# CPJKU/beat_this

Measured on AMD Instinct MI355X. Metric: audio-seconds processed/sec, higher is better.
Workload: dtype f32 activations, f16x3 products (3 x f16 MFMA on hi+lo operand halves, f32 accumulate); main-layer attention P.V: 2 x, probabilities as fp16 hi parts

## Files before the change

### beat_this_amd/_lib.py

```python
from __future__ import annotations

import ctypes as C
import os
import subprocess

import torch

PKG_DIR = os.path.dirname(os.path.abspath(__file__))
LIB_PATH = os.path.join(PKG_DIR, "libbeat_this_amd.so")
if os.environ.get("BT_DEV") == "1" and os.environ.get("BT_LIB_PATH"):
    LIB_PATH = os.environ["BT_LIB_PATH"]
SOURCES = ["gemm.hip", "gemm2.hip", "gemm3.hip", "gemm_mx8.hip", "attn.hip", "attn2.hip", "fused.hip", "fused2.hip", "qkv_front.hip", "frontend.hip", "logmel.hip",
           "tail.hip", "dbn.hip", "metrics.hip", "loss.hip", "data.hip", "train.hip", "train_front.hip", "optim.hip", "engine.hip"]
HEADERS = ["common.h", "chain.h", "kernels.h", "dropout.h", "train_common.h", "train_mixed.inc", "train_front_mixed.inc", "attn_x3_loop.inc", "attn_hq2_loop.inc", os.path.join("..", "..", "include", "beat_this_amd.h")]

BT_OK, BT_ERR_ARG, BT_ERR_HIP, BT_ERR_WORKSPACE = 0, -1, -2, -3
ABI_VERSION = 600
PREC_F32, PREC_HALF, PREC_F32X3 = 0, 1, 3
OPT_X3_ATTN_P16, OPT_X3_GEMM_FP8, OPT_WS_GUARD = 1, 2, 3
MAX_LAYERS = 32
PROFILE_CATEGORIES = ["stem", "qkv_gemm", "attn_flash", "out_gemm", "ff1_gemm", "ff2_gemm", "conv_gemm",
                      "linear_gemm", "head", "ff_fused", "attn_freq_fused", "layer_tail"]

GEMM_EPI_STORE, GEMM_EPI_RESID, GEMM_EPI_QKV = 0, 1, 2
# ... 183 lines not shown
    "bt_audio2beats_plan": (C.c_int, [C.c_void_p, C.c_int64, C.c_int, C.c_int, C.c_int, C.POINTER(A2BPlan)]),
    "bt_audio2beats_enqueue": (C.c_int, [C.c_void_p, C.c_void_p, C.c_int, C.POINTER(LogmelTables), C.c_void_p, C.c_int64, C.c_int, C.c_int,
                                         C.c_void_p, C.c_int, C.c_void_p, C.c_size_t, C.c_void_p, C.c_int]),
    "bt_profile_begin": (None, [C.c_void_p]),
    "bt_profile_end": (C.c_int, [C.c_void_p, C.c_void_p, C.c_void_p, C.c_int]),
    "bt_resample_batch": (C.c_int, [C.c_void_p, C.c_void_p, C.c_int, C.c_int64, C.c_int, C.c_int, C.c_void_p, C.c_int,
                                    C.c_void_p]),
    "bt_logmel_batch": (C.c_int, [C.c_void_p, C.POINTER(LogmelTables), C.c_void_p, C.c_int, C.c_int64, C.c_void_p]),
    "bt_split_chunks_batch": (C.c_int, [C.c_void_p, C.c_void_p, C.c_void_p, C.c_int, C.c_int, C.c_void_p]),
    "bt_aggregate_batch": (C.c_int, [C.c_void_p, C.c_void_p, C.c_void_p, C.c_void_p, C.c_void_p, C.c_int, C.c_int64,
                                     C.c_int, C.c_int, C.c_void_p, C.c_void_p]),
    "bt_peaks_batch": (C.c_int, [C.c_void_p, C.c_void_p, C.c_void_p, C.c_int, C.c_void_p, C.c_void_p]),
    "bt_peaks_host": (C.c_int, [C.c_void_p, C.c_int64, C.c_void_p, C.POINTER(C.c_int32)]),
    "bt_gemm": (C.c_int, [C.c_void_p, C.c_int, C.POINTER(GemmArgs)]),
    "bt_attention": (C.c_int, [C.c_void_p, C.c_int, C.POINTER(AttnArgs)]),
    "bt_gemm3": (C.c_int, [C.c_void_p, C.POINTER(Gemm3Args)]),
    "bt_gemm_mx8": (C.c_int, [C.c_void_p, C.c_void_p, C.c_void_p, C.c_void_p, C.c_void_p, C.c_void_p, C.c_int, C.c_int, C.c_int, C.c_int64]),
    "bt_attn_frag_blocks": (C.c_int, [C.c_int]),
    "bt_attention_frag": (C.c_int, [C.c_void_p, C.POINTER(AttnFragArgs)]),
    "bt_qkv_front": (C.c_int, [C.c_void_p, C.c_int, C.POINTER(PairWeights), C.c_void_p, C.c_void_p, C.c_int, C.c_int, C.c_int,
                               C.c_void_p, C.c_void_p, C.c_void_p, C.c_void_p, C.c_int]),
    "bt_outff_fused": (C.c_int, [C.c_void_p, C.c_int, C.POINTER(PairWeights), C.c_void_p, C.c_void_p, C.c_int64, C.c_void_p]),
    "bt_attnff_fused": (C.c_int, [C.c_void_p, C.c_int, C.POINTER(PairWeights), C.c_void_p, C.c_void_p, C.c_int64]),
    "bt_layer_tail": (C.c_int, [C.c_void_p, C.POINTER(PairWeights), C.c_int, C.c_void_p, C.c_void_p, C.c_int64, C.c_void_p,
                                C.c_void_p]),
    "bt_ff_fused": (C.c_int, [C.c_void_p, C.c_int, C.POINTER(PairWeights), C.c_void_p, C.c_int64]),
    "bt_dbn_tables": (C.c_int, [C.c_double, C.c_double, C.c_double, C.c_int, C.c_double, C.c_double, C.c_double, C.c_void_p,
                                C.c_int, C.c_void_p, C.POINTER(C.c_size_t)]),
    "bt_dbn_workspace_bytes": (C.c_size_t, [C.c_void_p, C.c_int, C.c_int64]),
    "bt_dbn_decode": (C.c_int, [C.c_void_p, C.c_void_p, C.c_void_p, C.c_void_p, C.c_int, C.c_void_p, C.c_int, C.c_int64,
                                C.c_void_p, C.c_void_p, C.c_size_t]),
    "bt_dbn_viterbi": (C.c_int, [C.c_void_p, C.c_void_p, C.c_void_p, C.c_int, C.c_void_p, C.c_int64, C.c_void_p, C.c_void_p,
                                 C.c_void_p, C.c_size_t]),
    "bt_dbn_viterbi_host": (C.c_int, [C.c_void_p, C.c_int, C.c_void_p, C.c_int64, C.c_void_p, C.c_void_p]),
    "bt_dbn_host": (C.c_int, [C.c_void_p, C.c_void_p, C.c_void_p, C.c_int64, C.c_void_p, C.POINTER(C.c_int32)]),
    "bt_dbn_host_act": (C.c_int, [C.c_void_p, C.c_void_p, C.c_int64, C.c_void_p, C.POINTER(C.c_int32)]),
    "bt_beat_metrics_workspace_bytes": (C.c_size_t, [C.c_int, C.c_int64, C.c_int64]),
    "bt_beat_metrics": (C.c_int, [C.c_void_p, C.c_void_p, C.c_void_p, C.c_void_p, C.c_void_p, C.c_int, C.c_double, C.c_double,
                                  C.c_double, C.c_double, C.c_double, C.c_void_p, C.c_size_t, C.c_void_p]),
    "bt_beat_metrics_host": (C.c_int, [C.c_void_p, C.c_void_p, C.c_void_p, C.c_void_p, C.c_int, C.c_double, C.c_double,
                                       C.c_double, C.c_double, C.c_double, C.c_void_p]),
    "bt_bce_loss_workspace_bytes": (C.c_size_t, [C.c_int, C.c_int64]),
    "bt_bce_loss": (C.c_int, [C.c_void_p, C.c_int, C.c_int, C.c_float, C.c_void_p, C.c_void_p, C.c_int, C.c_void_p, C.c_int,
                              C.c_void_p, C.c_int, C.c_void_p, C.c_int, C.c_int64, C.c_int64, C.c_void_p, C.c_size_t,
                              C.c_void_p, C.c_void_p, C.c_void_p, C.c_int, C.c_void_p, C.c_void_p]),
    "bt_bce_loss_backward": (C.c_int, [C.c_void_p, C.c_void_p, C.c_int64, C.c_void_p, C.c_int, C.c_int64, C.c_void_p, C.c_int]),
# ... 188 lines not shown
```

### beat_this_amd/csrc/engine.hip

```cpp
#include <algorithm>
#include <cmath>
#include <cstddef>
#include <cstdio>
#include <cstring>
#include <mutex>
#include <string>
#include <vector>

#include "../../include/beat_this_amd.h"
#include "common.h"
#include "kernels.h"


static thread_local std::string g_err;
static int bt_set_error(int code, const std::string& msg) {
  g_err = msg;
  return code;
}
int bt_set_error_external(int code, const char* msg) { return bt_set_error(code, msg); }

namespace prof {
struct Rec { int cat; hipEvent_t a, b; };
struct State { bool on = false; std::vector<Rec> recs; };
struct Scope {
// ... 2 lines not shown
    if (!st) return;
    Rec r; r.cat = cat;
    (void)hipEventCreate(&r.a); (void)hipEventCreate(&r.b);
    (void)hipEventRecord(r.a, s);
    idx = st->recs.size(); st->recs.push_back(r);
  }
  ~Scope() { if (st) (void)hipEventRecord(st->recs[idx].b, s); }
};
}

struct FwdGraph { int B, T, prec; void* ws; hipGraphExec_t exec; unsigned long stamp; };

struct bt_engine {
  bt_model_desc d;
  prof::State prof;
  std::mutex mu;
  std::vector<FwdGraph> graphs;
  unsigned long graph_clock = 0;
  hipStream_t cap_stream = nullptr;
  std::vector<int> warm;
  int x3_attn_p16 = 1;
  int x3_gemm_fp8 = 0;
  int ws_guard = 0;
};
enum { CAT_STEM = 0, CAT_QKV, CAT_ATTN_FLASH, CAT_OUT, CAT_FF1, CAT_FF2, CAT_CONV, CAT_LINEAR,
       CAT_HEAD, CAT_FF_FUSED, CAT_ATTN_FREQ_FUSED, CAT_LAYER_TAIL, CAT_COUNT };

namespace {

inline size_t align_up(size_t v, size_t a) { return (v + a - 1) / a * a; }

struct Workspace {
  float* xa; float* xb; float* xm; float* gates; void* xmb;
  void* qkv; void* ao; void* hid;
  void* qf; void* kf; void* vf; float* gates_h; int nbp;
  float* ssq[2];
  int* status;
  int* fix_mask;
  size_t total;
};

Workspace carve(char* base, int B, int T, int D, int ff_mult, int prec, size_t guard = 0,
                std::vector<int64_t>* regions = nullptr) {
  const bool x3 = prec == BT_PREC_F32X3;
  if (x3) prec = BT_PREC_F32;
  const size_t es = prec == BT_PREC_F32 ? 4 : 2;
  const size_t bt = (size_t)B * T;
// ... 414 lines not shown
  *out = e;
  return BT_OK;
}
static void drop_graphs(bt_engine* e) {
  for (auto& g : e->graphs) (void)hipGraphExecDestroy(g.exec);
  e->graphs.clear();
  e->warm.clear();
}
void bt_engine_destroy(bt_engine* e) {
  if (!e) return;
  for (auto& r : e->prof.recs) { (void)hipEventDestroy(r.a); (void)hipEventDestroy(r.b); }
  drop_graphs(e);
  if (e->cap_stream) (void)hipStreamDestroy(e->cap_stream);
  delete e;
}

int bt_engine_set_option(bt_engine* e, int option, int value) {
  if (!e) return bt_set_error(BT_ERR_ARG, "null argument");
  std::lock_guard<std::mutex> lock(e->mu);
  if (option == BT_OPT_X3_ATTN_P16 && value >= 0 && value <= 3) { if (e->x3_attn_p16 != value) drop_graphs(e); e->x3_attn_p16 = value; return BT_OK; }
  if (option == BT_OPT_X3_GEMM_FP8 && value >= 0 && value <= 2) { if (e->x3_gemm_fp8 != value) drop_graphs(e); e->x3_gemm_fp8 = value; return BT_OK; }
  if (option == BT_OPT_WS_GUARD && value >= 0 && value % 256 == 0) { if (e->ws_guard != value) drop_graphs(e); e->ws_guard = value; return BT_OK; }
  return bt_set_error(BT_ERR_ARG, "unknown engine option / value");
}
int bt_engine_get_option(const bt_engine* e, int option, int* value) {
  if (!e || !value) return bt_set_error(BT_ERR_ARG, "null argument");
  if (option == BT_OPT_X3_ATTN_P16) { *value = e->x3_attn_p16; return BT_OK; }
  if (option == BT_OPT_X3_GEMM_FP8) { *value = e->x3_gemm_fp8; return BT_OK; }
  if (option == BT_OPT_WS_GUARD) { *value = e->ws_guard; return BT_OK; }
  return bt_set_error(BT_ERR_ARG, "unknown engine option");
}

size_t bt_workspace_bytes(const bt_engine* e, int B, int T, int prec) {
  if (!e || B <= 0 || T <= 0) return 0;
  return carve(nullptr, B, T, e->d.transformer_dim, e->d.ff_mult, prec, (size_t)e->ws_guard).total;
}

int bt_workspace_regions(const bt_engine* e, int B, int T, int prec, int64_t* begin_end, int max) {
  if (!e || B <= 0 || T <= 0 || max < 0 || (max > 0 && !begin_end)) return bt_set_error(BT_ERR_ARG, "bad argument to bt_workspace_regions");
  if (prec != BT_PREC_F32 && prec != BT_PREC_HALF && prec != BT_PREC_F32X3) return bt_set_error(BT_ERR_ARG, "unknown precision");
  std::vector<int64_t> r;
  carve(nullptr, B, T, e->d.transformer_dim, e->d.ff_mult, prec, (size_t)e->ws_guard, &r);
  const int n = (int)(r.size() / 2);
  for (int i = 0; i < std::min(n, max); ++i) { begin_end[2 * i] = r[2 * i]; begin_end[2 * i + 1] = r[2 * i + 1]; }
  return n;
}
// ... 314 lines not shown
  size_t off = 0;
  auto take = [&](size_t bytes) { size_t o = off; off += align_up(bytes, 256); return o; };
  plan->forward_bytes = bt_workspace_bytes(e, plan->B, plan->T, prec);
  plan->off_forward = take(plan->forward_bytes);
  plan->off_chunks = take((size_t)plan->B * plan->T * 128 * 4);
  plan->off_chunk_logits = take((size_t)2 * plan->B * plan->T * 4);
  plan->off_wave22 = take(up == down ? 0 : (size_t)n22 * 4);
  plan->off_spect = take((size_t)n * 128 * 4);
  plan->off_logits = take((size_t)2 * n * 4);
  plan->off_result = take((size_t)plan->result_words * 4);
  plan->ws_bytes = off;
  return BT_OK;
}

int bt_audio2beats_enqueue(bt_engine* e, void* stream, int prec, const bt_logmel_tables* t, const float* d_audio, int64_t n_in,
                           int up, int down, const float* d_filter, int half_len, void* d_ws, size_t ws_bytes, int32_t* h_result,
                           int use_graph) {
  if (!e || !t || !d_audio || !d_ws || !h_result) return bt_set_error(BT_ERR_ARG, "null argument");
  if (up != down && (!d_filter || half_len < 0)) return bt_set_error(BT_ERR_ARG, "resampling needs the polyphase filter");
  bt_a2b_plan pl;
  if (int rc = bt_audio2beats_plan(e, n_in, up, down, prec, &pl)) return rc;
  if (pl.ws_bytes > ws_bytes) return bt_set_error(BT_ERR_WORKSPACE, "workspace too small (bt_audio2beats_plan)");
  std::lock_guard<std::mutex> lock(e->mu);
  const int max_T = e->d.rope_len > 0 ? e->d.rope_len : 1536;
  if (pl.T > max_T) return bt_set_error(BT_ERR_ARG, "chunk longer than the rotary table");
  hipStream_t s = (hipStream_t)stream;
  char* ws = (char*)d_ws;
  float* wave22 = (float*)(ws + pl.off_wave22);
  float* spect = (float*)(ws + pl.off_spect);
  float* chunks = (float*)(ws + pl.off_chunks);
  float* cb = (float*)(ws + pl.off_chunk_logits);
  float* cd = cb + (size_t)pl.B * pl.T;
  float* beat = (float*)(ws + pl.off_logits);
  float* downb = beat + pl.n_frames;
  int32_t* res = (int32_t*)(ws + pl.off_result);
  void* fws = ws + pl.off_forward;
  const int border = 6;
  const float* a22 = d_audio;
  if (up != down) {
    const bt_span_t one{d_audio, (long)n_in, 0, (long)pl.n22};
    LAUNCH(launch_resample(one, nullptr, 1, (long)pl.n22, up, down, d_filter, half_len, wave22, s), "resample");
    a22 = wave22;
  }
  LogmelP lp;
  fill_logmel(lp, t, spect);
  lp.one = bt_span_t{a22, (long)pl.n22, 0, (long)pl.n_frames};
// ... 202 lines not shown
```

### beat_this_amd/csrc/fused2.hip

```cpp
#include <type_traits>

#include "chain.h"
#include "kernels.h"

namespace {

typedef __amdgpu_buffer_rsrc_t rsrc_t;
typedef __attribute__((address_space(3))) void* lptr_t;
DEVI unsigned pk2_hf(float a, float b) {
  const hfx2 t = {(hf)a, (hf)b};
  return __builtin_bit_cast(unsigned, t);
}

template <typename T, int C>
struct WRing {
  static constexpr int KT = C / 32;
  static constexpr int TILE_B = 32 * 32 * (int)sizeof(T);
  static constexpr int STEP_B = 2 * KT * TILE_B;
#ifndef BT_F2_NST_HL128
#define BT_F2_NST_HL128 2
#endif
#ifndef BT_F2_NST_HL64
#define BT_F2_NST_HL64 2
#endif
  static constexpr bool HL = sizeof(T) == 4 && !std::is_same<T, float>::value;
  static constexpr int NST = C == 128 ? (HL ? BT_F2_NST_HL128 : 3) : (HL && C == 64 ? BT_F2_NST_HL64 : 4);
  static constexpr int CH = STEP_B / 4096;
  rsrc_t rs;
  char* lds;
  int tid, wave, total;
  DEVI void issue(int s) {
    if (s >= total) return;
    char* dst = lds + (s % NST) * STEP_B + wave * 1024;
#pragma unroll
    for (int i = 0; i < CH; ++i)
      __builtin_amdgcn_raw_ptr_buffer_load_lds(rs, (lptr_t)(dst + i * 4096), 16, tid * 16, s * STEP_B + i * 4096, 0, 0);
  }
  DEVI void prologue() {
#pragma unroll
    for (int s = 0; s < NST - 1; ++s) issue(s);
  }
  DEVI const char* acquire(int s) {
    const int ahead = min(NST - 2, total - 1 - s);
    if (ahead >= 2) asm volatile("s_waitcnt vmcnt(%0) lgkmcnt(0)" ::"n"(2 * CH) : "memory");
    else if (ahead == 1) asm volatile("s_waitcnt vmcnt(%0) lgkmcnt(0)" ::"n"(CH) : "memory");
    else asm volatile("s_waitcnt vmcnt(0) lgkmcnt(0)" ::: "memory");
    __builtin_amdgcn_s_barrier();
    issue(s + NST - 1);
    return lds + (s % NST) * STEP_B;
  }
};

template <typename T, int C, bool STORE_X = true>
DEVI void ff_tail(WRing<T, C>& ws, int step0, float (&xn)[C / 32][16], const float* b1s, const float* b2,
                  float* xrow, hf* xbrow, bool ok, int lane, int g) {
  constexpr int KT = C / 32, HB = 4 * C / 32;
  constexpr int TILE_B = WRing<T, C>::TILE_B;
  float ss = 0.f;
#pragma unroll
  for (int kt = 0; kt < KT; ++kt)
#pragma unroll
    for (int r = 0; r < 16; ++r) ss = fmaf(xn[kt][r], xn[kt][r], ss);
  ss += __shfl_xor(ss, 32);
  constexpr float PW = OpScale<T>::PW;
  const float scale = sqrtf((float)C) / fmaxf(sqrtf(ss), 1e-12f) * PW;
  Frag<T> xf[KT];
#pragma unroll
  for (int kt = 0; kt < KT; ++kt) xf[kt] = pack_frag<T>(xn[kt]);
  f32x16 acc2[KT];
#pragma unroll
  for (int mt = 0; mt < KT; ++mt)
#pragma unroll
    for (int r = 0; r < 16; ++r) acc2[mt][r] = xn[mt][r] * (1.f / PW);
#pragma unroll 1
  for (int hb = 0; hb < HB; ++hb) {
    const char* wb = ws.acquire(step0 + hb);
    f32x16 acc1;
    zero16(acc1);
#pragma unroll
    for (int kt = 0; kt < KT; ++kt) mma32(acc1, lds_frag<T>(wb + kt * TILE_B, lane), xf[kt]);
    float h[16];
#pragma unroll
    for (int a = 0; a < 4; ++a) {
      const f32x4 b = *reinterpret_cast<const f32x4*>(b1s + hb * 32 + 8 * a + 4 * g);
#pragma unroll
      for (int j = 0; j < 4; ++j) h[4 * a + j] = gelu_t<T>(fmaf(acc1[4 * a + j], scale, b[j]));
    }
    const Frag<T> hf = pack_frag<T>(h);
#pragma unroll
    for (int mt = 0; mt < KT; ++mt) mma32(acc2[mt], lds_frag<T>(wb + (KT + mt) * TILE_B, lane), hf);
  }
#pragma unroll
  for (int mt = 0; mt < KT; ++mt) {
    f32x4 v[4];
#pragma unroll
    for (int a = 0; a < 4; ++a) {
      const int f0 = mt * 32 + 8 * a + 4 * g;
      const f32x4 b = *reinterpret_cast<const f32x4*>(b2 + f0);
#pragma unroll
      for (int j = 0; j < 4; ++j) v[a][j] = fmaf(acc2[mt][4 * a + j], PW, b[j]);
      if constexpr (STORE_X) {
        if (ok) *reinterpret_cast<f32x4*>(xrow + f0) = v[a];
      }
    }
    if (xbrow) {
      typedef __attribute__((ext_vector_type(4))) unsigned int u32x4;
      if constexpr (std::is_same<T, hl>::value) {
#pragma unroll
        for (int k = 0; k < 2; ++k) {
          unsigned xh[2], xl[2], yh[2], yl[2];
#pragma unroll
          for (int i = 0; i < 2; ++i) {
            split_hl4(v[2 * k][2 * i], v[2 * k][2 * i + 1], v[2 * k + 1][2 * i], v[2 * k + 1][2 * i + 1], xh[i], xl[i], yh[i], yl[i]);
// ... 1 lines not shown
          auto h0 = __builtin_amdgcn_permlane32_swap(xh[0], yh[0], false, false);
          auto h1 = __builtin_amdgcn_permlane32_swap(xh[1], yh[1], false, false);
          auto l0 = __builtin_amdgcn_permlane32_swap(xl[0], yl[0], false, false);
          auto l1 = __builtin_amdgcn_permlane32_swap(xl[1], yl[1], false, false);
          if (ok) {
            *reinterpret_cast<u32x4*>(xbrow + mt * 64 + 16 * k + 8 * g) = u32x4{h0[0], h1[0], h0[1], h1[1]};
            *reinterpret_cast<u32x4*>(xbrow + mt * 64 + 32 + 16 * k + 8 * g) = u32x4{l0[0], l1[0], l0[1], l1[1]};
          }
        }
      } else {
#pragma unroll
      for (int k = 0; k < 2; ++k) {
        const unsigned x0 = pk2_hf(v[2 * k][0], v[2 * k][1]), x1 = pk2_hf(v[2 * k][2], v[2 * k][3]);
        const unsigned y0 = pk2_hf(v[2 * k + 1][0], v[2 * k + 1][1]), y1 = pk2_hf(v[2 * k + 1][2], v[2 * k + 1][3]);
        auto r0 = __builtin_amdgcn_permlane32_swap(x0, y0, false, false);
        auto r1 = __builtin_amdgcn_permlane32_swap(x1, y1, false, false);
        if (ok) *reinterpret_cast<u32x4*>(xbrow + mt * 32 + 16 * k + 8 * g) = u32x4{r0[0], r1[0], r0[1], r1[1]};
      }
      }
    }
  }
}

template <typename T, int C, bool STORE_X = true>
__global__ __launch_bounds__(256) void outff_fused_kernel(const FusedOutFFP p) {
  constexpr int KT = C / 32, HB = 4 * C / 32;
  constexpr int TILE_B = WRing<T, C>::TILE_B, STEP_B = WRing<T, C>::STEP_B, NST = WRing<T, C>::NST;
  __shared__ __attribute__((aligned(16))) char wl[NST * STEP_B + 4 * C * 4];
  float* b1s = reinterpret_cast<float*>(wl + NST * STEP_B);
  const int tid = threadIdx.x, lane = tid & 63, wave = __builtin_amdgcn_readfirstlane(tid >> 6);
  const int g = lane >> 5, lr = lane & 31;
  const long tok = ((long)blockIdx.x * 4 + wave) * 32 + lr;
  const bool ok = tok < p.M;
  float* xrow = p.x + (ok ? tok : 0) * C;
  for (int i = tid; i < 4 * C; i += 256) b1s[i] = p.b1[i];

  const T* arow = reinterpret_cast<const T*>(p.ao) + (ok ? tok : 0) * C;
  Frag<T> af[KT];
#pragma unroll
  for (int kt = 0; kt < KT; ++kt) af[kt] = ldg_frag<T>(arow + kt * 32 + 16 * g);
  float xn[KT][16];
#pragma unroll
  for (int mt = 0; mt < KT; ++mt)
#pragma unroll
    for (int a = 0; a < 4; ++a) {
      const f32x4 v = ok ? *reinterpret_cast<const f32x4*>(xrow + mt * 32 + 8 * a + 4 * g) : f32x4{0.f, 0.f, 0.f, 0.f};
#pragma unroll
      for (int j = 0; j < 4; ++j) xn[mt][4 * a + j] = v[j];
    }
  WRing<T, C> ws;
  ws.rs = __builtin_amdgcn_make_buffer_rsrc(const_cast<void*>(p.wfrag), 0, (unsigned)((KT + HB) * STEP_B), 0x00020000);
  ws.lds = wl; ws.tid = tid; ws.wave = wave; ws.total = KT + HB;
  __syncthreads();
  asm volatile("s_waitcnt vmcnt(0)" ::: "memory");
  ws.prologue();
#pragma unroll
  for (int mt = 0; mt < KT; ++mt) {
    const char* wb = ws.acquire(mt);
    f32x16 acc;
    zero16(acc);
#pragma unroll
    for (int kt = 0; kt < KT; ++kt) mma32(acc, lds_frag<T>(wb + kt * TILE_B, lane), af[kt]);
#pragma unroll
    for (int r = 0; r < 16; ++r) xn[mt][r] = fmaf(acc[r], OpScale<T>::PW, xn[mt][r]);
  }
  hf* xbrow = p.xb ? reinterpret_cast<hf*>(p.xb) + tok * C * (std::is_same<T, hl>::value ? 2 : 1) : nullptr;
  ff_tail<T, C, STORE_X>(ws, KT, xn, b1s, p.b2, xrow, xbrow, ok, lane, g);
}

template <typename T, int C>
__global__ __launch_bounds__(256) void attnff_fused_kernel(const FusedAttnFFP p) {
  constexpr int KT = C / 32;
  constexpr int H = C / 32;
  constexpr int F = 1024 / C;
  constexpr int HB = 4 * C / 32;
  constexpr int TILE_B = WRing<T, C>::TILE_B, STEP_B = WRing<T, C>::STEP_B, NST = WRing<T, C>::NST;
  __shared__ __attribute__((aligned(16))) char wl[NST * STEP_B + 4 * C * 4];
  float* b1s = reinterpret_cast<float*>(wl + NST * STEP_B);
  const int tid = threadIdx.x, lane = tid & 63, wave = __builtin_amdgcn_readfirstlane(tid >> 6);
  const int g = lane >> 5, lr = lane & 31;
  const long tok = ((long)blockIdx.x * 4 + wave) * 32 + lr;
  const bool ok = tok < p.M;
  float* xrow = p.x + (ok ? tok : 0) * C;
  for (int i = tid; i < 4 * C; i += 256) b1s[i] = p.b1[i];

  float ss = 0.f;
  Frag<T> xf[KT];
#pragma unroll
  for (int kt = 0; kt < KT; ++kt) xf[kt] = ldx_frag<T>(xrow + kt * 32 + 16 * g, ok, ss);
  ss += __shfl_xor(ss, 32);
  constexpr float PW = OpScale<T>::PW, PA = OpScale<T>::PA;
  const float scale = sqrtf((float)C) / fmaxf(sqrtf(ss), 1e-12f) * PW;
  float sk[16];
#pragma unroll
  for (int r = 0; r < 16; ++r) sk[r] = __shfl(scale, crow(r, g));
  const int pos = (int)(tok & (F - 1));
  f32x2 cs[8];
#pragma unroll
  for (int a = 0; a < 4; ++a)
#pragma unroll
    for (int b = 0; b < 2; ++b)
      cs[2 * a + b] = *reinterpret_cast<const f32x2*>(p.rope + ((long)pos * 16 + 4 * a + 2 * g + b) * 2);
  float bg[H];
#pragma unroll
  for (int hd = 0; hd < H; ++hd) bg[hd] = p.b_gates[hd];
  WRing<T, C> ws;
  ws.rs = __builtin_amdgcn_make_buffer_rsrc(const_cast<void*>(p.wfrag), 0, (unsigned)((1 + 2 * H + HB) * STEP_B), 0x00020000);
  ws.lds = wl; ws.tid = tid; ws.wave = wave; ws.total = 1 + 2 * H + HB;
  __syncthreads();
  asm volatile("s_waitcnt vmcnt(0)" ::: "memory");
  ws.prologue();

  float gate[H];
  {
    const char* wb = ws.acquire(0);
    f32x16 ag;
    zero16(ag);
#pragma unroll
    for (int kt = 0; kt < KT; ++kt) mma32(ag, lds_frag<T>(wb + kt * TILE_B, lane), xf[kt]);
#pragma unroll
    for (int hd = 0; hd < H; ++hd) {
      float v = __shfl(ag[hd], lr);
      gate[hd] = sigmoidf(fmaf(v, scale, bg[hd]));
    }
  }

  f32x16 acco[KT];
#pragma unroll
  for (int mt = 0; mt < KT; ++mt) zero16(acco[mt]);
// ... 57 lines not shown
      float o[16];
#pragma unroll
      for (int r = 0; r < 16; ++r) o[r] = ao[r] * fin;
      const Frag<T> of = pack_frag<T>(o);
#pragma unroll
      for (int mt = 0; mt < KT; ++mt) mma32(acco[mt], lds_frag<T>(wb + (KT + mt) * TILE_B, lane), of);
    }
  }
  f32x4 xv[KT][4];
#pragma unroll
  for (int mt = 0; mt < KT; ++mt)
#pragma unroll
    for (int a = 0; a < 4; ++a)
      xv[mt][a] = ok ? *reinterpret_cast<const f32x4*>(xrow + mt * 32 + 8 * a + 4 * g) : f32x4{0.f, 0.f, 0.f, 0.f};
  asm volatile("s_waitcnt vmcnt(0)" ::: "memory");
  __builtin_amdgcn_sched_barrier(0);
  float xn[KT][16];
#pragma unroll
  for (int mt = 0; mt < KT; ++mt)
#pragma unroll
    for (int a = 0; a < 4; ++a)
#pragma unroll
      for (int j = 0; j < 4; ++j) xn[mt][4 * a + j] = fmaf(acco[mt][4 * a + j], PW, xv[mt][a][j]);
  ff_tail<T, C>(ws, 1 + 2 * H, xn, b1s, p.b2, xrow, nullptr, ok, lane, g);
}

template <typename T>
int launch_outff_t(const FusedOutFFP& p, hipStream_t s) {
  dim3 grid((unsigned)((p.M + 127) / 128)), block(256);
  if constexpr (std::is_same<T, hl>::value) {
    if (p.shadow_only) {
      if (!p.xb) return -2;
      switch (p.C) {
        case 64: hipLaunchKernelGGL((outff_fused_kernel<T, 64, false>), grid, block, 0, s, p); break;
        case 128: hipLaunchKernelGGL((outff_fused_kernel<T, 128, false>), grid, block, 0, s, p); break;
        default: return -2;
      }
      return (int)hipGetLastError();
    }
  } else if (p.shadow_only) {
    return -2;
  }
  switch (p.C) {
    case 32: hipLaunchKernelGGL((outff_fused_kernel<T, 32>), grid, block, 0, s, p); break;
    case 64: hipLaunchKernelGGL((outff_fused_kernel<T, 64>), grid, block, 0, s, p); break;
    case 128: hipLaunchKernelGGL((outff_fused_kernel<T, 128>), grid, block, 0, s, p); break;
    default: return -2;
  }
  return (int)hipGetLastError();
}
template <typename T>
int launch_attnff_t(const FusedAttnFFP& p, hipStream_t s) {
  dim3 grid((unsigned)((p.M + 127) / 128)), block(256);
  switch (p.C) {
    case 32: hipLaunchKernelGGL((attnff_fused_kernel<T, 32>), grid, block, 0, s, p); break;
    case 64: hipLaunchKernelGGL((attnff_fused_kernel<T, 64>), grid, block, 0, s, p); break;
    case 128: hipLaunchKernelGGL((attnff_fused_kernel<T, 128>), grid, block, 0, s, p); break;
    default: return -2;
  }
  return (int)hipGetLastError();
}

}

int launch_outff_fused(const FusedOutFFP& p, int prec, hipStream_t s) {
  if (p.M <= 0) return -2;
  if (prec == BT_PREC_F32X3) return BT_HALF_IS_BF16 ? -2 : launch_outff_t<hl>(p, s);
  return prec == BT_PREC_F32 ? launch_outff_t<float>(p, s) : launch_outff_t<hf>(p, s);
}
int launch_attnff_fused(const FusedAttnFFP& p, int prec, hipStream_t s) {
  if (p.M <= 0) return -2;
  if (prec == BT_PREC_F32X3) return BT_HALF_IS_BF16 ? -2 : launch_attnff_t<hl>(p, s);
  return prec == BT_PREC_F32 ? launch_attnff_t<float>(p, s) : launch_attnff_t<hf>(p, s);
}
```

### beat_this_amd/csrc/kernels.h

```cpp
#pragma once
#include <hip/hip_runtime.h>
#include <stdint.h>

#ifndef BT_PREC_F32
#define BT_PREC_F32 0
#define BT_PREC_HALF 1
#endif
#ifndef BT_PREC_F32X3
#define BT_PREC_F32X3 3
#endif

enum {
  GEMM_EPI_STORE = 0,
  GEMM_EPI_RESID = 1,
  GEMM_EPI_QKV = 2
};
enum {
  GEMM_F_RMS = 1,
  GEMM_F_BIAS = 2,
  GEMM_F_GELU = 4,
  GEMM_F_OUT_F32 = 8,
  GEMM_F_A_F32 = 16,
  GEMM_F_CONV = 32,
  GEMM_F_ROWMAP = 64
// ... 96 lines not shown
  float* x; long M; int C;
  const void* wfrag;
  const float* b1; const float* b2;
  void* xb;
};
int launch_ff_fused(const FusedFFP& p, int prec, hipStream_t s);

struct FusedOutFFP {
  float* x; long M; int C;
  const void* ao;
  const void* wfrag;
  const float* b1; const float* b2;
  void* xb;
  int shadow_only;
};
int launch_outff_fused(const FusedOutFFP& p, int prec, hipStream_t s);
struct FusedAttnFFP {
  float* x; long M; int C;
  const float* b_gates; const float* rope;
  const void* wfrag;
  const float* b1; const float* b2;
};
int launch_attnff_fused(const FusedAttnFFP& p, int prec, hipStream_t s);

struct LayerTailP {
  float* x; long M; int C; int hidden;
  const void* ao;
  const void* wfrag;
  const float* b1; const float* b2;
  void* xb;
  float* ssq_out;
};
bool layer_tail_supported(int C, int hidden);
int launch_layer_tail(const LayerTailP& p, hipStream_t s);

struct StemP {
  const float* spect;
  float* x;
  const float* bn1_scale; const float* bn1_shift;
  const float* w;
  const float* bias;
  int B, T;
};
int launch_stem(const StemP& p, hipStream_t s);

struct HeadP {
// ... 37 lines not shown
```

### beat_this_amd/pack.py

```python
from __future__ import annotations

import collections
import ctypes as C
import math
import threading

import torch

from . import _lib, tables

LOG2E = 1.4426950408889634
BN_EPS = 1e-5


def perm32(w: torch.Tensor) -> torch.Tensor:
    idx = torch.tensor([(r & 3) + 8 * (r >> 2) + 4 * g for g in range(2) for r in range(16)])
    n, k = w.shape
    return w.reshape(n, k // 32, 32)[:, :, idx].reshape(n, k).contiguous()


def fragment_tiles(w: torch.Tensor) -> torch.Tensor:
    r, k = w.shape
    t = w.reshape(r // 32, 32, k // 32, 2, 16)
    return t.permute(0, 2, 3, 1, 4).reshape(r // 32, k // 32, 64, 16)
# ... 256 lines not shown
            t = tail_fragment_major(sd[pa + "to_out.0.weight"].to(torch.float32), perm32(w1),
                                    perm32(sd[pf + "net.4.weight"].to(torch.float32)))
            t = t.to(_lib.half_torch_dtype()).to(self.device)
            self._keep.append(t)
            pw.w_tail_frag = t.data_ptr()


class PackedPair:

    def __init__(self, sd: dict, attn_prefix: str, ff_prefix: str, dim: int, device):
        self.device = torch.device(device)
        self._keep: list[torch.Tensor] = []
        self.weights = _lib.PairWeights()
        sd = {k: v.detach().to("cpu", torch.float32) for k, v in sd.items()}
        PackedModel._pair(self, self.weights, sd, attn_prefix, ff_prefix, dim, x3=True)

    _f32 = PackedModel._f32
    _mat = PackedModel._mat
    _hl32 = PackedModel._hl32
    _hl8 = PackedModel._hl8
    _x3_stream = PackedModel._x3_stream


class Engine:

    def __init__(self, packed: PackedModel):
        self.packed = packed
        self.device = packed.device
        h = C.c_void_p()
        _lib.check(_lib.lib().bt_engine_create(C.byref(packed.desc), C.byref(h)))
        self._h = h
        self._ws = collections.OrderedDict()
        self._graphs = collections.OrderedDict()
        self._graph_ws = {}
        self._a2b_ws = {}
        self._graphs_ok = True
        self.profiling = False
        self._lock = threading.Lock()
        self.last_fallbacks = 0

    def __del__(self):
        try:
            if getattr(self, "_h", None):
                _lib.lib().bt_engine_destroy(self._h)
                self._h = None
        except Exception:
            pass

    MAX_WORKSPACES = 4
    SHRINK_AFTER = 8
    OPTIONS = {"x3_attn_p16": 1, "x3_gemm_fp8": 2, "ws_guard": 3}

    def set_options(self, opts: dict) -> None:
        for name in opts:
            if name not in self.OPTIONS:
                raise ValueError(f"unknown engine option {name!r} (known: {sorted(self.OPTIONS)})")
        if int(opts.get("x3_gemm_fp8", 0)) > 0:
# ... 103 lines not shown
    def forward_unit(self, x: torch.Tensor, prec: int, unit: int, index: int, out_shape) -> torch.Tensor:
        _lib.require_gpu(x, "sub-module input")
        B, T = int(x.shape[0]), int(x.shape[1])
        if B == 0 or T == 0:
            raise ValueError("empty batch")
        if prec == _lib.PREC_F32X3:
            prec = _lib.PREC_F32
        x = x.to(torch.float32).contiguous()
        self.ensure_positions(T)
        ws = self._workspace(_lib.lib().bt_workspace_bytes(self._h, B, T, prec))
        out = torch.empty(tuple(out_shape), dtype=torch.float32, device=self.device)
        with torch.cuda.device(self.device):
            _lib.check(_lib.lib().bt_forward_unit(self._h, _lib.stream_ptr(self.device), prec, unit, index, x.data_ptr(),
                                                  out.data_ptr(), B, T, ws.data_ptr(), ws.numel()))
        return out

    GRAPH_MAX_CHUNKS = 11
    GRAPH_T = 1500
    GRAPH_MAX_ENTRIES = 12

    def graph_forward(self, B: int, T: int, prec: int):
        if not self._graphs_ok or T != self.GRAPH_T or B > self.GRAPH_MAX_CHUNKS or self.profiling:
            return None
        stream = torch.cuda.current_stream(self.device)
        key = (stream, B, T, prec)
        e = self._graphs.pop(key, None)
        if e is None:
            try:
                e = _GraphEntry(self, B, T, prec, stream)
            except Exception as err:
                self._graphs_ok = False
                self._graph_error = repr(err)
                return None
        cache = self._graphs
        cache[key] = e
        while len(cache) > self.GRAPH_MAX_ENTRIES:
            cache.popitem(last=False)
        return e

    def _graph_workspace(self, stream, need: int) -> torch.Tensor:
        pool = self._graph_ws
        ws = pool.get(stream)
        if ws is None or ws.numel() < need:
            ws = pool[stream] = torch.empty(need, dtype=torch.uint8, device=self.device)
        return ws

# ... 67 lines not shown
```

### include/beat_this_amd.h

```cpp
#ifndef BEAT_THIS_AMD_H
#define BEAT_THIS_AMD_H
#include <stddef.h>
#include <stdint.h>

#ifdef __cplusplus
extern "C" {
#endif

#define BT_OK 0
#define BT_ERR_ARG (-1)
#define BT_ERR_HIP (-2)
#define BT_ERR_WORKSPACE (-3)

#define BT_PREC_F32 0
#define BT_PREC_HALF 1

#define BT_PREC_F32X3 3

#define BT_MAX_LAYERS 32

typedef struct bt_engine bt_engine;

typedef struct {
  int32_t dim, heads;
// ... 232 lines not shown
  int32_t n_seq, L, heads, inner, nbp, o_div; int64_t o_outer, o_inner, o_tok;
  int32_t x3, out_f32; int32_t* status;
  int32_t* scratch;
} bt_attn_frag_args;
int bt_gemm_mx8(void* stream, const void* d_A, const void* d_SA, const void* d_W, const void* d_SW, float* d_out, int M, int N,
                int K, int64_t ldo);

typedef struct {
  const void* A; int64_t lda; int32_t M, K; const void* W; int32_t N, epi; const float* bias;
  const float* ssq_in; int32_t ssq_parts; void* out; int64_t ldo; float* x; int64_t ldx; void* xb; float* ssq_out;
  int32_t n_seq, L, nbp, heads; const float* rope; void* qf; void* kf; void* vf; float* gates; const float* b_gates;
  int32_t no_resid;
  int32_t gelu, conv_C2, conv_T, conv_F;
  int32_t x3; int32_t* status;
} bt_gemm3_args;
int bt_gemm3(void* stream, const bt_gemm3_args* a);
int bt_attn_frag_blocks(int L);
int bt_attention_frag(void* stream, const bt_attn_frag_args* a);
int bt_qkv_front(void* stream, int prec, const bt_pair_weights* w, const float* d_rope, const float* d_x, int B, int T, int F,
                 void* d_q, void* d_k, void* d_v, float* d_gates, int nbp);
int bt_ff_fused(void* stream, int prec, const bt_pair_weights* w, float* d_x, int64_t M);
int bt_outff_fused(void* stream, int prec, const bt_pair_weights* w, const void* d_ao, float* d_x, int64_t M, void* d_xb);
int bt_attnff_fused(void* stream, int prec, const bt_pair_weights* w, const float* d_rope, float* d_x, int64_t M);
int bt_layer_tail(void* stream, const bt_pair_weights* w, int hidden, const void* d_ao, float* d_x, int64_t M, void* d_xb,
                  float* d_ssq_out);

#define BT_TRAIN_UNIT_HEAD 16
#define BT_TRAIN_DW_ROWS 1024
#define BT_TRAIN_CS_ROWS 64
#define BT_TRAIN_ATTN_BLOCK 64
typedef struct {
  int32_t B, T, dim, hidden, rope_len, residual, sum_head, reserved;
  const float* rope;
  const float* gamma; const float* w1; const float* b1; const float* w2; const float* b2; const float* w3;
  const float* x; float* y; float* y2; float* save_o; float* save_lse;
  const float* gy; const float* gy2;
  float* gx; float* g_gamma; float* g_w1; float* g_b1; float* g_w2; float* g_b2; float* g_w3;
  void* ws; size_t ws_bytes;
} bt_train_args;
void bt_train_struct_sizes(int32_t* out);
size_t bt_train_workspace_bytes(int unit, int backward, int B, int T, int dim, int hidden);
int bt_train_forward(void* stream, int unit, const bt_train_args* a);
int bt_train_backward(void* stream, int unit, const bt_train_args* a);

#define BT_DROP_ATTN_P 0
#define BT_DROP_ATTN_OUT 1
// ... 95 lines not shown
```

Before: 63380.

## Software-pipeline FF tail in fused attn+FF kernel, overlapping GELU with next MFMA

Adds a skewed variant of the fused FF tail for hi/lo x3 operands. The first-layer MFMA for hidden block hb+1 is interleaved with the GELU/bias epilogue of block hb, and one extra LDS weight-ring stage is added so the prefetch distance is kept. By default it is enabled only for the C=64 attention+FF fused kernel; a runtime mask toggles the other variants and invalidates captured graphs. The aim is to hide the VALU epilogue behind MFMA work. The cost is more LDS and more registers, which could lower occupancy.

```diff
diff --git a/beat_this_amd/_lib.py b/beat_this_amd/_lib.py
--- a/beat_this_amd/_lib.py
+++ b/beat_this_amd/_lib.py
@@ -229,6 +229,7 @@
                                C.c_void_p, C.c_void_p, C.c_void_p, C.c_void_p, C.c_int]),
     "bt_outff_fused": (C.c_int, [C.c_void_p, C.c_int, C.POINTER(PairWeights), C.c_void_p, C.c_void_p, C.c_int64, C.c_void_p]),
     "bt_attnff_fused": (C.c_int, [C.c_void_p, C.c_int, C.POINTER(PairWeights), C.c_void_p, C.c_void_p, C.c_int64]),
+    "bt_fused2_set_pipeline": (C.c_int, [C.c_int]),
     "bt_layer_tail": (C.c_int, [C.c_void_p, C.POINTER(PairWeights), C.c_int, C.c_void_p, C.c_void_p, C.c_int64, C.c_void_p,
                                 C.c_void_p]),
     "bt_ff_fused": (C.c_int, [C.c_void_p, C.c_int, C.POINTER(PairWeights), C.c_void_p, C.c_int64]),
diff --git a/beat_this_amd/csrc/engine.hip b/beat_this_amd/csrc/engine.hip
--- a/beat_this_amd/csrc/engine.hip
+++ b/beat_this_amd/csrc/engine.hip
@@ -1,4 +1,5 @@
 #include <algorithm>
+#include <atomic>
 #include <cmath>
 #include <cstddef>
 #include <cstdio>
@@ -48,7 +49,9 @@
   int x3_attn_p16 = 1;
   int x3_gemm_fp8 = 0;
   int ws_guard = 0;
+  unsigned f2_epoch = 0;
 };
+static std::atomic<unsigned> g_f2_epoch{0};
 enum { CAT_STEM = 0, CAT_QKV, CAT_ATTN_FLASH, CAT_OUT, CAT_FF1, CAT_FF2, CAT_CONV, CAT_LINEAR,
        CAT_HEAD, CAT_FF_FUSED, CAT_ATTN_FREQ_FUSED, CAT_LAYER_TAIL, CAT_COUNT };
 
@@ -509,6 +512,11 @@
   if (option == BT_OPT_X3_GEMM_FP8 && value >= 0 && value <= 2) { if (e->x3_gemm_fp8 != value) drop_graphs(e); e->x3_gemm_fp8 = value; return BT_OK; }
   if (option == BT_OPT_WS_GUARD && value >= 0 && value % 256 == 0) { if (e->ws_guard != value) drop_graphs(e); e->ws_guard = value; return BT_OK; }
   return bt_set_error(BT_ERR_ARG, "unknown engine option / value");
+}
+int bt_fused2_set_pipeline(int mask) {
+  const int before = fused2_set_pipeline(mask);
+  if (before != fused2_pipeline()) ++g_f2_epoch;
+  return before;
 }
 int bt_engine_get_option(const bt_engine* e, int option, int* value) {
   if (!e || !value) return bt_set_error(BT_ERR_ARG, "null argument");
@@ -869,6 +877,7 @@
   if (int rc = bt_audio2beats_plan(e, n_in, up, down, prec, &pl)) return rc;
   if (pl.ws_bytes > ws_bytes) return bt_set_error(BT_ERR_WORKSPACE, "workspace too small (bt_audio2beats_plan)");
   std::lock_guard<std::mutex> lock(e->mu);
+  if (const unsigned ep = g_f2_epoch.load(); ep != e->f2_epoch) { drop_graphs(e); e->f2_epoch = ep; }
   const int max_T = e->d.rope_len > 0 ? e->d.rope_len : 1536;
   if (pl.T > max_T) return bt_set_error(BT_ERR_ARG, "chunk longer than the rotary table");
   hipStream_t s = (hipStream_t)stream;
diff --git a/beat_this_amd/csrc/fused2.hip b/beat_this_amd/csrc/fused2.hip
--- a/beat_this_amd/csrc/fused2.hip
+++ b/beat_this_amd/csrc/fused2.hip
@@ -1,3 +1,4 @@
+#include <atomic>
 #include <type_traits>
 
 #include "chain.h"
@@ -12,8 +13,15 @@
   return __builtin_bit_cast(unsigned, t);
 }
 
+enum { F2_PIPE_ATTNFF32 = 1, F2_PIPE_OUTFF32 = 2, F2_PIPE_ATTNFF64 = 4, F2_PIPE_OUTFF64 = 8 };
+#ifndef BT_F2_PIPE
+#define BT_F2_PIPE F2_PIPE_ATTNFF64
+#endif
 template <typename T, int C>
+constexpr bool f2_can_pipe = C <= 64 && std::is_same<T, hl>::value;
+template <typename T, int C, bool PIPE = false>
 struct WRing {
+  static_assert(!PIPE || f2_can_pipe<T, C>, "the skewed FF tail exists for (hi, lo) operands at C = 32 / 64 only");
   static constexpr int KT = C / 32;
   static constexpr int TILE_B = 32 * 32 * (int)sizeof(T);
   static constexpr int STEP_B = 2 * KT * TILE_B;
@@ -24,7 +32,13 @@
 #define BT_F2_NST_HL64 2
 #endif
   static constexpr bool HL = sizeof(T) == 4 && !std::is_same<T, float>::value;
-  static constexpr int NST = C == 128 ? (HL ? BT_F2_NST_HL128 : 3) : (HL && C == 64 ? BT_F2_NST_HL64 : 4);
+#ifndef BT_F2_NST_HL32P
+#define BT_F2_NST_HL32P 4
+#endif
+  static constexpr int NST0 = C == 128 ? (HL ? BT_F2_NST_HL128 : 3) : (HL && C == 64 ? BT_F2_NST_HL64 : 4);
+  static constexpr int NST = !PIPE ? NST0 : C == 32 ? BT_F2_NST_HL32P : NST0 + 1;
+  static constexpr int DIST = NST - 1 - (PIPE ? 1 : 0);
+  static_assert(DIST >= 1 && DIST <= 3, "the counted waits of acquire cover at most two steps in flight");
   static constexpr int CH = STEP_B / 4096;
   rsrc_t rs;
   char* lds;
@@ -38,24 +52,25 @@
   }
   DEVI void prologue() {
 #pragma unroll
-    for (int s = 0; s < NST - 1; ++s) issue(s);
-  }
+    for (int s = 0; s < DIST; ++s) issue(s);
+  }
+  DEVI const char* stage(int s) const { return lds + (s % NST) * STEP_B; }
   DEVI const char* acquire(int s) {
-    const int ahead = min(NST - 2, total - 1 - s);
+    const int ahead = min(DIST - 1, total - 1 - s);
     if (ahead >= 2) asm volatile("s_waitcnt vmcnt(%0) lgkmcnt(0)" ::"n"(2 * CH) : "memory");
     else if (ahead == 1) asm volatile("s_waitcnt vmcnt(%0) lgkmcnt(0)" ::"n"(CH) : "memory");
     else asm volatile("s_waitcnt vmcnt(0) lgkmcnt(0)" ::: "memory");
     __builtin_amdgcn_s_barrier();
-    issue(s + NST - 1);
-    return lds + (s % NST) * STEP_B;
+    issue(s + DIST);
+    return stage(s);
   }
 };
 
-template <typename T, int C, bool STORE_X = true>
-DEVI void ff_tail(WRing<T, C>& ws, int step0, float (&xn)[C / 32][16], const float* b1s, const float* b2,
+template <typename T, int C, bool STORE_X = true, bool PIPE = false>
+DEVI void ff_tail(WRing<T, C, PIPE>& ws, int step0, float (&xn)[C / 32][16], const float* b1s, const float* b2,
                   float* xrow, hf* xbrow, bool ok, int lane, int g) {
   constexpr int KT = C / 32, HB = 4 * C / 32;
-  constexpr int TILE_B = WRing<T, C>::TILE_B;
+  constexpr int TILE_B = WRing<T, C, PIPE>::TILE_B;
   float ss = 0.f;
 #pragma unroll
   for (int kt = 0; kt < KT; ++kt)
@@ -72,13 +87,7 @@
   for (int mt = 0; mt < KT; ++mt)
 #pragma unroll
     for (int r = 0; r < 16; ++r) acc2[mt][r] = xn[mt][r] * (1.f / PW);
-#pragma unroll 1
-  for (int hb = 0; hb < HB; ++hb) {
-    const char* wb = ws.acquire(step0 + hb);
-    f32x16 acc1;
-    zero16(acc1);
-#pragma unroll
-    for (int kt = 0; kt < KT; ++kt) mma32(acc1, lds_frag<T>(wb + kt * TILE_B, lane), xf[kt]);
+  auto ff2 = [&](int hb, const char* wb, const f32x16& acc1) {
     float h[16];
 #pragma unroll
     for (int a = 0; a < 4; ++a) {
@@ -89,6 +98,61 @@
     const Frag<T> hf = pack_frag<T>(h);
 #pragma unroll
     for (int mt = 0; mt < KT; ++mt) mma32(acc2[mt], lds_frag<T>(wb + (KT + mt) * TILE_B, lane), hf);
+  };
+  if constexpr (!PIPE) {
+#pragma unroll 1
+    for (int hb = 0; hb < HB; ++hb) {
+      const char* wb = ws.acquire(step0 + hb);
+      f32x16 acc1;
+      zero16(acc1);
+#pragma unroll
+      for (int kt = 0; kt < KT; ++kt) mma32(acc1, lds_frag<T>(wb + kt * TILE_B, lane), xf[kt]);
+      ff2(hb, wb, acc1);
+    }
+  } else {
+    static_assert(HB % 2 == 0 && HB >= 4, "");
+    f32x16 a0, a1;
+    auto both = [&](int hb, f32x16& next, const f32x16& cur) {
+      const char* w1 = ws.acquire(step0 + hb + 1);
+      const char* w2 = ws.stage(step0 + hb);
+      Frag<T> wf[KT];
+      wf[0] = lds_frag<T>(w1, lane);
+      zero16(next);
+      constexpr int IA[6] = {2, 3, 0, 1, 0, 1}, IB[6] = {0, 1, 2, 3, 0, 1};
+      float h[16];
+      f32x4 b[4];
+#pragma unroll
+      for (int e = 0; e < 16; ++e) {
+        if (e % 4 == 0) b[e / 4] = *reinterpret_cast<const f32x4*>(b1s + hb * 32 + 8 * (e / 4) + 4 * g);
+#pragma unroll
+        for (int kt = 1; kt < KT; ++kt)
+          if (e == kt * 16 / KT - 2) wf[kt] = lds_frag<T>(w1 + kt * TILE_B, lane);
+        float c = cur[e];
+        if (e == 0) asm volatile("" : "+v"(c), "+v"(next));
+        else asm volatile("" : "+v"(c), "+v"(h[e - 1]), "+v"(next));
+#pragma unroll
+        for (int i = e * 6 * KT / 16; i < (e + 1) * 6 * KT / 16; ++i)
+          next = MFMA32_H(wf[i / 6].v[IA[i % 6]], xf[i / 6].v[IB[i % 6]], next);
+        h[e] = gelu_t<T>(fmaf(c, scale, b[e / 4][e % 4]));
+        __builtin_amdgcn_sched_barrier(0);
+      }
+      const Frag<T> hf = pack_frag<T>(h);
+#pragma unroll
+      for (int mt = 0; mt < KT; ++mt) mma32(acc2[mt], lds_frag<T>(w2 + (KT + mt) * TILE_B, lane), hf);
+    };
+    {
+      const char* wb = ws.acquire(step0);
+      zero16(a0);
+#pragma unroll
+      for (int kt = 0; kt < KT; ++kt) mma32(a0, lds_frag<T>(wb + kt * TILE_B, lane), xf[kt]);
+    }
+#pragma unroll 1
+    for (int hb = 0; hb < HB - 2; hb += 2) {
+      both(hb, a1, a0);
+      both(hb + 1, a0, a1);
+    }
+    both(HB - 2, a1, a0);
+    ff2(HB - 1, ws.stage(step0 + HB - 1), a1);
   }
 #pragma unroll
   for (int mt = 0; mt < KT; ++mt) {
@@ -136,10 +200,10 @@
   }
 }
 
-template <typename T, int C, bool STORE_X = true>
+template <typename T, int C, bool STORE_X = true, bool PIPE = false>
 __global__ __launch_bounds__(256) void outff_fused_kernel(const FusedOutFFP p) {
   constexpr int KT = C / 32, HB = 4 * C / 32;
-  constexpr int TILE_B = WRing<T, C>::TILE_B, STEP_B = WRing<T, C>::STEP_B, NST = WRing<T, C>::NST;
+  constexpr int TILE_B = WRing<T, C, PIPE>::TILE_B, STEP_B = WRing<T, C, PIPE>::STEP_B, NST = WRing<T, C, PIPE>::NST;
   __shared__ __attribute__((aligned(16))) char wl[NST * STEP_B + 4 * C * 4];
   float* b1s = reinterpret_cast<float*>(wl + NST * STEP_B);
   const int tid = threadIdx.x, lane = tid & 63, wave = __builtin_amdgcn_readfirstlane(tid >> 6);
@@ -162,7 +226,7 @@
 #pragma unroll
       for (int j = 0; j < 4; ++j) xn[mt][4 * a + j] = v[j];
     }
-  WRing<T, C> ws;
+  WRing<T, C, PIPE> ws;
   ws.rs = __builtin_amdgcn_make_buffer_rsrc(const_cast<void*>(p.wfrag), 0, (unsigned)((KT + HB) * STEP_B), 0x00020000);
   ws.lds = wl; ws.tid = tid; ws.wave = wave; ws.total = KT + HB;
   __syncthreads();
@@ -179,16 +243,16 @@
     for (int r = 0; r < 16; ++r) xn[mt][r] = fmaf(acc[r], OpScale<T>::PW, xn[mt][r]);
   }
   hf* xbrow = p.xb ? reinterpret_cast<hf*>(p.xb) + tok * C * (std::is_same<T, hl>::value ? 2 : 1) : nullptr;
-  ff_tail<T, C, STORE_X>(ws, KT, xn, b1s, p.b2, xrow, xbrow, ok, lane, g);
-}
-
-template <typename T, int C>
+  ff_tail<T, C, STORE_X, PIPE>(ws, KT, xn, b1s, p.b2, xrow, xbrow, ok, lane, g);
+}
+
+template <typename T, int C, bool PIPE = false>
 __global__ __launch_bounds__(256) void attnff_fused_kernel(const FusedAttnFFP p) {
   constexpr int KT = C / 32;
   constexpr int H = C / 32;
   constexpr int F = 1024 / C;
   constexpr int HB = 4 * C / 32;
-  constexpr int TILE_B = WRing<T, C>::TILE_B, STEP_B = WRing<T, C>::STEP_B, NST = WRing<T, C>::NST;
+  constexpr int TILE_B = WRing<T, C, PIPE>::TILE_B, STEP_B = WRing<T, C, PIPE>::STEP_B, NST = WRing<T, C, PIPE>::NST;
   __shared__ __attribute__((aligned(16))) char wl[NST * STEP_B + 4 * C * 4];
   float* b1s = reinterpret_cast<float*>(wl + NST * STEP_B);
   const int tid = threadIdx.x, lane = tid & 63, wave = __builtin_amdgcn_readfirstlane(tid >> 6);
@@ -218,7 +282,7 @@
   float bg[H];
 #pragma unroll
   for (int hd = 0; hd < H; ++hd) bg[hd] = p.b_gates[hd];
-  WRing<T, C> ws;
+  WRing<T, C, PIPE> ws;
   ws.rs = __builtin_amdgcn_make_buffer_rsrc(const_cast<void*>(p.wfrag), 0, (unsigned)((1 + 2 * H + HB) * STEP_B), 0x00020000);
   ws.lds = wl; ws.tid = tid; ws.wave = wave; ws.total = 1 + 2 * H + HB;
   __syncthreads();
@@ -322,13 +386,24 @@
     for (int a = 0; a < 4; ++a)
 #pragma unroll
       for (int j = 0; j < 4; ++j) xn[mt][4 * a + j] = fmaf(acco[mt][4 * a + j], PW, xv[mt][a][j]);
-  ff_tail<T, C>(ws, 1 + 2 * H, xn, b1s, p.b2, xrow, nullptr, ok, lane, g);
-}
+  ff_tail<T, C, true, PIPE>(ws, 1 + 2 * H, xn, b1s, p.b2, xrow, nullptr, ok, lane, g);
+}
+
+constexpr int F2_PIPE_ALL = F2_PIPE_ATTNFF32 | F2_PIPE_OUTFF32 | F2_PIPE_ATTNFF64 | F2_PIPE_OUTFF64;
+std::atomic<int> g_f2_pipe{(BT_F2_PIPE) & F2_PIPE_ALL};
 
 template <typename T>
 int launch_outff_t(const FusedOutFFP& p, hipStream_t s) {
   dim3 grid((unsigned)((p.M + 127) / 128)), block(256);
   if constexpr (std::is_same<T, hl>::value) {
+    const int pipe = g_f2_pipe.load(std::memory_order_relaxed);
+    if ((p.C == 32 && (pipe & F2_PIPE_OUTFF32)) || (p.C == 64 && (pipe & F2_PIPE_OUTFF64))) {
+      if (p.shadow_only && (!p.xb || p.C != 64)) return -2;
+      if (p.shadow_only) hipLaunchKernelGGL((outff_fused_kernel<T, 64, false, true>), grid, block, 0, s, p);
+      else if (p.C == 64) hipLaunchKernelGGL((outff_fused_kernel<T, 64, true, true>), grid, block, 0, s, p);
+      else hipLaunchKernelGGL((outff_fused_kernel<T, 32, true, true>), grid, block, 0, s, p);
+      return (int)hipGetLastError();
+    }
     if (p.shadow_only) {
       if (!p.xb) return -2;
       switch (p.C) {
@@ -352,6 +427,14 @@
 template <typename T>
 int launch_attnff_t(const FusedAttnFFP& p, hipStream_t s) {
   dim3 grid((unsigned)((p.M + 127) / 128)), block(256);
+  if constexpr (std::is_same<T, hl>::value) {
+    const int pipe = g_f2_pipe.load(std::memory_order_relaxed);
+    if ((p.C == 32 && (pipe & F2_PIPE_ATTNFF32)) || (p.C == 64 && (pipe & F2_PIPE_ATTNFF64))) {
+      if (p.C == 32) hipLaunchKernelGGL((attnff_fused_kernel<T, 32, true>), grid, block, 0, s, p);
+      else hipLaunchKernelGGL((attnff_fused_kernel<T, 64, true>), grid, block, 0, s, p);
+      return (int)hipGetLastError();
+    }
+  }
   switch (p.C) {
     case 32: hipLaunchKernelGGL((attnff_fused_kernel<T, 32>), grid, block, 0, s, p); break;
     case 64: hipLaunchKernelGGL((attnff_fused_kernel<T, 64>), grid, block, 0, s, p); break;
@@ -363,6 +446,8 @@
 
 }
 
+int fused2_pipeline() { return g_f2_pipe.load(std::memory_order_relaxed); }
+int fused2_set_pipeline(int mask) { return g_f2_pipe.exchange(mask < 0 ? (BT_F2_PIPE) & F2_PIPE_ALL : mask & F2_PIPE_ALL); }
 int launch_outff_fused(const FusedOutFFP& p, int prec, hipStream_t s) {
   if (p.M <= 0) return -2;
   if (prec == BT_PREC_F32X3) return BT_HALF_IS_BF16 ? -2 : launch_outff_t<hl>(p, s);
diff --git a/beat_this_amd/csrc/kernels.h b/beat_this_amd/csrc/kernels.h
--- a/beat_this_amd/csrc/kernels.h
+++ b/beat_this_amd/csrc/kernels.h
@@ -142,6 +142,8 @@
   const float* b1; const float* b2;
 };
 int launch_attnff_fused(const FusedAttnFFP& p, int prec, hipStream_t s);
+int fused2_pipeline();
+int fused2_set_pipeline(int mask);
 
 struct LayerTailP {
   float* x; long M; int C; int hidden;
diff --git a/beat_this_amd/pack.py b/beat_this_amd/pack.py
--- a/beat_this_amd/pack.py
+++ b/beat_this_amd/pack.py
@@ -302,6 +302,19 @@
     _x3_stream = PackedModel._x3_stream
 
 
+_f2_epoch = 0
+
+
+F2_ATTNFF32, F2_OUTFF32, F2_ATTNFF64, F2_OUTFF64, F2_ALL = 1, 2, 4, 8, 15
+
+
+def set_fused2_pipeline(mask: int) -> int:
+    global _f2_epoch
+    before = int(_lib.lib().bt_fused2_set_pipeline(int(mask)))
+    _f2_epoch += 1
+    return before
+
+
 class Engine:
 
     def __init__(self, packed: PackedModel):
@@ -313,6 +326,7 @@
         self._ws = collections.OrderedDict()
         self._graphs = collections.OrderedDict()
         self._graph_ws = {}
+        self._graph_epoch = _f2_epoch
         self._a2b_ws = {}
         self._graphs_ok = True
         self.profiling = False
@@ -462,6 +476,9 @@
     def graph_forward(self, B: int, T: int, prec: int):
         if not self._graphs_ok or T != self.GRAPH_T or B > self.GRAPH_MAX_CHUNKS or self.profiling:
             return None
+        if self._graph_epoch != _f2_epoch:
+            self._drop_graphs()
+            self._graph_epoch = _f2_epoch
         stream = torch.cuda.current_stream(self.device)
         key = (stream, B, T, prec)
         e = self._graphs.pop(key, None)
diff --git a/include/beat_this_amd.h b/include/beat_this_amd.h
--- a/include/beat_this_amd.h
+++ b/include/beat_this_amd.h
@@ -278,6 +278,12 @@
 int bt_ff_fused(void* stream, int prec, const bt_pair_weights* w, float* d_x, int64_t M);
 int bt_outff_fused(void* stream, int prec, const bt_pair_weights* w, const void* d_ao, float* d_x, int64_t M, void* d_xb);
 int bt_attnff_fused(void* stream, int prec, const bt_pair_weights* w, const float* d_rope, float* d_x, int64_t M);
+#define BT_F2_ATTNFF32 1
+#define BT_F2_OUTFF32 2
+#define BT_F2_ATTNFF64 4
+#define BT_F2_OUTFF64 8
+#define BT_F2_ALL 15
+int bt_fused2_set_pipeline(int mask);
 int bt_layer_tail(void* stream, const bt_pair_weights* w, int hidden, const void* d_ao, float* d_x, int64_t M, void* d_xb,
                   float* d_ssq_out);
 
```

After: 63480 (median of 2 runs). No clear change (+0.1%).
